# THUDM/GCC

Measured on NVIDIA H100. Metric: subgraphs/sec (MoCo pretrain step), higher is better.
Workload: dtype f32

## Files before the change

gcc_b200/csrc/posenc.cu:

```cuda
#include "common.cuh"

#include <stdlib.h>

namespace gccb {

#define GCCB_EIG_MAXSWEEP 14
#define GCCB_CF_B 48
#ifndef GCCB_CF_DEG0
#define GCCB_CF_DEG0 8
#endif
#ifndef GCCB_CF_DEG
#define GCCB_CF_DEG 16
#endif
#define GCCB_CF_LOGGAIN 19.1138f
#define GCCB_CF_MARGIN 0.05f
#define GCCB_CF_MARGIN_BELOW 0.25f
#ifndef GCCB_CF_SWEEPS0
#define GCCB_CF_SWEEPS0 0
#endif
#ifndef GCCB_CF_SWEEPS0_CLUSTER
#define GCCB_CF_SWEEPS0_CLUSTER 1
#endif
#define GCCB_DN_A 96
#define GCCB_DN_B 144
#define GCCB_DN_C 228
#define GCCB_CF_NSM 160
#define GCCB_CF_NSM_C 384
#define GCCB_CF_NSM_D1 1536
#define GCCB_CF_NSM_D 3584
#ifndef GCCB_CAP_MID2
#define GCCB_CAP_MID2 (GCCB_NUM_SMS * 2)
#endif
#ifndef GCCB_CAP_DN_A
#define GCCB_CAP_DN_A (GCCB_NUM_SMS * 4)
#endif
#ifndef GCCB_CAP_DN_B
#define GCCB_CAP_DN_B (GCCB_NUM_SMS * 2)
#endif
#ifndef GCCB_CAP_DN_C
#define GCCB_CAP_DN_C GCCB_NUM_SMS
#endif
#ifndef GCCB_BIG_NT
#define GCCB_BIG_NT 512
#endif
#define GCCB_CF_MAXIT 8
#define GCCB_GS_PANEL 4
#define GCCB_CF_TOL 4.0e-5f
#define GCCB_CF_STAG 2.0e-3f

#ifdef GCCB_EMU
#define GCCB_CLK() 0ll
#else
#define GCCB_CLK() clock64()
#endif
#define GCCB_TICK(k) do { if (threadIdx.x == 0) { long long t_ = GCCB_CLK(); ph[k] += t_ - t_last; t_last = t_; } } while (0)

#define GCCB_EIG_NCLASS 8
__device__ __forceinline__ int eig_class(int n, int dense_max) {
  if (n <= dense_max) return n <= GCCB_DN_A ? 0 : n <= GCCB_DN_B ? 1 : 2;
  return n <= GCCB_CF_NSM ? 3 : n <= GCCB_CF_NSM_C ? 4 : n <= GCCB_CF_NSM_D1 ? 5 : n <= GCCB_CF_NSM_D ? 6 : 7;
}

__global__ void __launch_bounds__(256)
posenc_classify_kernel(const int64_t* __restrict__ counters, const int32_t* __restrict__ node_off,
                       int B, int dense_max, int32_t* __restrict__ worklist, int32_t* __restrict__ counts) {
  __shared__ int scan_scratch[33];
  const int tid = threadIdx.x;
  int base[GCCB_EIG_NCLASS] = {0};
  for (int s0 = 0; s0 < 2 * B; s0 += 256) {
    int slot = s0 + tid;
    int cls = -1;
    if (slot < 2 * B) {
      int view = slot / B;
      if (node_off[view * (B + 1) + B] >= 0) cls = eig_class((int)counters[(size_t)slot * 4], dense_max);
    }
#pragma unroll
    for (int c = 0; c < GCCB_EIG_NCLASS; ++c) {
      int tot;
      int ex = block_scan_excl(cls == c ? 1 : 0, scan_scratch, &tot);
      if (cls == c) worklist[(size_t)c * 2 * B + base[c] + ex] = slot;
      base[c] += tot;
    }
  }
  if (tid < GCCB_EIG_NCLASS) counts[tid] = base[tid];
}

template <int NT>
__device__ __forceinline__ int jacobi_ritz48(float* A, float* V, float* cs , int* pq , int LD,
                                              float tol, int max_sweeps, long long* n_work = nullptr,
                                              long long* n_idle = nullptr) {
  constexpr int M = GCCB_CF_B, HALF = M / 2;
  const int tid = threadIdx.x;
  __shared__ float4 rec2[2][HALF];
  __shared__ int nrot2[2];
  (void)cs; (void)pq;
  for (int idx = tid; idx < M * M; idx += NT) {
    const int j = idx / M, i = idx - j * M;
    V[j * LD + i] = i == j ? 1.0f : 0.f;
  }
  __syncthreads();
  int sweep = 0;
  for (; sweep < max_sweeps; ++sweep) {
    if (max_sweeps > 1) {
      int any = 0;
      for (int idx = tid; idx < M * M; idx += NT) {
        const int q = idx / M, p = idx - q * M;
        if (p < q && fabsf(A[q * LD + p]) > tol * 0.5f * (fabsf(A[p * LD + p]) + fabsf(A[q * LD + q]))) any = 1;
// ... 990 lines not shown
    }
    if (tid == 0) {
      float w = 0.f, lo = theta[0], tk = theta[0];
      for (int c = 0; c < k; ++c) { w = fmaxf(w, resid[c]); tk = fminf(tk, theta[c]); }
      for (int i = 1; i < CB; ++i) lo = fminf(lo, theta[i]);
      if (tk < GCCB_CF_MARGIN_BELOW) lo = fminf(lo, tk - GCCB_CF_MARGIN);
      s_bc[0] = sqrtf(w);
      s_bc[1] = lo;
    }
    __syncthreads();
    const float w_all = s_bc[0];
    converged = (w_all < GCCB_CF_TOL) || (iter >= 2 && w_all < GCCB_CF_STAG && w_all > 0.5f * prev_worst);
    prev_worst = w_all;
    cut = fminf(fmaxf(s_bc[1], -0.9f), 0.95f);
    __syncthreads();
    GCCB_TICK(5);
  }
  if (C.rank == 0 && tid == 0) {
    if (!converged) atomicOr(flags, (int)GCCB_FLAG_EIG_NOCONV);
    dbg_iters[slot] = iter; dbg_res[slot] = prev_worst;
    for (int i = 0; i < 8; ++i) dbg_phase[(size_t)slot * 8 + i] = ph[i];
  }
  if (eigvals && C.rank == 0)
    for (int c = tid; c < pos_dim; c += NT) eigvals[(size_t)slot * pos_dim + c] = c < k ? theta[k - 1 - c] : 0.f;
  {
    float* best = part;
    for (int c = warp; c < k; c += NW) {
      float bb = -1.f, bval = 0.f; int brow = 0x7fffffff;
      for (int rl = lane; rl < nloc; rl += 32) {
        float x = X[(size_t)rl * ld + (k - 1 - c)], a = fabsf(x);
        if (a > bb) { bb = a; brow = r_lo + rl; bval = x; }
      }
#pragma unroll
      for (int o = 16; o > 0; o >>= 1) {
        float ob = __shfl_xor_sync(0xffffffffu, bb, o);
        int orow = __shfl_xor_sync(0xffffffffu, brow, o);
        float ov = __shfl_xor_sync(0xffffffffu, bval, o);
        if (ob > bb || (ob == bb && orow < brow)) { bb = ob; brow = orow; bval = ov; }
      }
      if (lane == 0) { best[c] = bb; best[48 + c] = __int_as_float(brow); best[96 + c] = bval; }
    }
    cl_sync<CS>();
    for (int c = tid; c < k; c += NT) {
      float bb = -1.f, bval = 0.f; int brow = 0x7fffffff;
      for (int q = 0; q < CS; ++q) {
        const float* rb = cl_map<CS>(best, q);
        float ob = rb[c]; int orow = __float_as_int(rb[48 + c]); float ov = rb[96 + c];
        if (ob > bb || (ob == bb && orow < brow)) { bb = ob; brow = orow; bval = ov; }
      }
      sgn[c] = bval < 0.f ? -1.0f : 1.0f;
    }
    __syncthreads();
  }
  float* out = pos + ((size_t)view * node_cap + noff) * pos_dim;
  for (int rl = warp; rl < nloc; rl += NW) {
    float u = 0.f;
    if (lane < k) u = sgn[lane] * X[(size_t)rl * ld + (k - 1 - lane)];
    if (normalize) {
      float ss = warp_sum(u * u);
      if (ss > 0.f) u = u / sqrtf(ss);
    }
    if (lane < pos_dim) out[(size_t)(r_lo + rl) * pos_dim + lane] = u;
  }
  cl_sync<CS>();
  }
}

#ifndef GCCB_DN_INVIT
#define GCCB_DN_INVIT 3
#endif
#ifndef GCCB_DN_MGS
#define GCCB_DN_MGS 1
#endif
#define GCCB_DN_PIVMIN 1.0e-30f
#define GCCB_DN_GUARD 1.0e-9f
#define GCCB_DN_TIGHT 2.0e-6f
#define GCCB_DN_DELTA 4.0e-6f
#define GCCB_DN_GAPTOL 1.0e-2f
#define GCCB_DN_RES_FLAG 1.0e-3f


__host__ __device__ constexpr int dn_ld(int n) { return ((n + 23) / 32) * 32 + 8; }

__device__ __forceinline__ int dn_sturm(const float* __restrict__ d, const float* __restrict__ e2, int n, float x) {
  float q = d[0] - x;
  if (fabsf(q) < GCCB_DN_PIVMIN) q = -GCCB_DN_PIVMIN;
  int c = q < 0.f ? 1 : 0;
  for (int i = 1; i < n; ++i) {
    q = (d[i] - x) - __fdividef(e2[i - 1], q);
    if (fabsf(q) < GCCB_DN_PIVMIN) q = -GCCB_DN_PIVMIN;
    c += q < 0.f ? 1 : 0;
  }
  return c;
}

template <int NMAX, int NT>
__device__ __forceinline__ void posenc_dense_item(const int slot, int B, int node_cap, int edge_cap,
                    const int32_t* __restrict__ node_off, const int32_t* __restrict__ b_indptr,
                    const int32_t* __restrict__ b_indices, const int32_t* __restrict__ sub_deg, int pos_dim, int normalize,
                    float* __restrict__ blocks, float* __restrict__ pos, float* __restrict__ eigvals,
                    int32_t* __restrict__ flags, int32_t* __restrict__ dbg_iters, float* __restrict__ dbg_res,
                    long long* __restrict__ dbg_phase) {
  constexpr int NW = NT / 32, NP = ((NMAX + 3) & ~3) + 4, NR = (NMAX + 31) / 32, CPW = 32 / NW;
  static_assert(NT >= 2 * NMAX && NW <= 32 && 32 % NW == 0, "two threads per matrix row");
  GCCB_DYN_SMEM(float, A);
  __align__(16) __shared__ float d[NP];
  __align__(16) __shared__ float e[NP];
  __align__(16) __shared__ float e2[NP];
  __align__(16) __shared__ float taus[NP];
  __align__(16) __shared__ float vbuf[NP];
  __align__(16) __shared__ float pbuf[NP];
  __align__(16) __shared__ float xbuf[NP];
  __align__(16) __shared__ float dinv[NP];
  __shared__ float ztail[32 * 32];
  __shared__ float lam[32], lamp[32], lo[32], hi[32], sgn[32];
  __shared__ int cnt[NT];
  __shared__ float part[NW * 32];
  long long ph[8] = {0, 0, 0, 0, 0, 0, 0, 0}, t_last = GCCB_CLK();
  const int view = slot / B, g = slot - view * B;
  const int noff = node_off[view * (B + 1) + g];
  const int n = node_off[view * (B + 1) + g + 1] - noff;
  const int tid = threadIdx.x, lane = tid & 31, warp = tid >> 5;
  const int k = min(n - 2, pos_dim);
  float* out = pos + ((size_t)view * node_cap + noff) * pos_dim;
  if (k <= 0) {
    for (int i = tid; i < n * pos_dim; i += NT) out[i] = 0.f;
    if (eigvals)
      for (int i = tid; i < pos_dim; i += NT) eigvals[(size_t)slot * pos_dim + i] = 0.f;
    if (tid == 0) { dbg_iters[slot] = 0; dbg_res[slot] = 0.f; }
    return;
  }
  const int ld = dn_ld(n);
  const int zb = n > 32 ? n - 32 : 0;
  auto zrow = [&](int i) -> float* { return i < zb ? A + (size_t)i * ld + (n - 32) : ztail + (i - zb) * 32; };
  const int32_t* v_indptr = b_indptr + (size_t)view * (node_cap + 1);
  const int32_t* v_indices = b_indices + (size_t)view * edge_cap;
  const int32_t* v_deg = sub_deg + (size_t)view * node_cap;
  float* U0 = blocks + ((size_t)view * node_cap + noff) * (GCCB_CF_B + 1);
  float* U1 = U0 + (size_t)2 * node_cap * (GCCB_CF_B + 1);
  for (int i = tid; i < NP; i += NT) { d[i] = 0.f; e[i] = 0.f; e2[i] = 0.f; taus[i] = 0.f; vbuf[i] = 0.f; pbuf[i] = 0.f; xbuf[i] = 0.f; }
  for (int i = tid; i < n; i += NT) {
    int dg = v_deg[noff + i];
    dinv[i] = 1.0f / sqrtf((float)(dg < 1 ? 1 : dg));
  }
  {
    float4* A4 = reinterpret_cast<float4*>(A);
    for (int i = tid; i < n * ld / 4; i += NT) A4[i] = make_float4(0.f, 0.f, 0.f, 0.f);
  }
  __syncthreads();
  for (int i = warp; i < n; i += NW) {
    const int beg = v_indptr[noff + i], end = v_indptr[noff + i + 1];
    const float di = dinv[i];
    for (int ed = beg + lane; ed < end; ed += 32) {
      int j = v_indices[ed] - noff;
      atomicAdd(&A[(size_t)j * ld + i], di * dinv[j]);
    }
  }
  __syncthreads();
  for (int i = tid; i < n; i += NT) xbuf[i] = i >= 1 ? A[(size_t)i * ld] : 0.f;
  __syncthreads();
  GCCB_TICK(0);
  {
    const int r = tid >> 1, h = tid & 1;
    float* row = A + (size_t)r * ld;
    for (int kk = 0; kk + 2 < n; ++kk) {
      const int c0 = (kk + 1) & ~3;
      const bool mine = r > kk && r < n;
      if (warp * 16 + 15 <= kk || warp * 16 >= n) {
        __syncthreads();
        __syncthreads();
        continue;
      }
      float y = 0.f;
      if (mine) {
        float y0 = 0.f, y1 = 0.f;
        int c = c0 + 4 * h;
        for (; c + 8 < n; c += 16) {
          const float4 a = *reinterpret_cast<const float4*>(row + c);
          const float4 x = *reinterpret_cast<const float4*>(xbuf + c);
          const float4 a2 = *reinterpret_cast<const float4*>(row + c + 8);
          const float4 x2 = *reinterpret_cast<const float4*>(xbuf + c + 8);
          y0 = fmaf(a.x, x.x, y0);
          y1 = fmaf(a.y, x.y, y1);
          y0 = fmaf(a.z, x.z, y0);
          y1 = fmaf(a.w, x.w, y1);
          y0 = fmaf(a2.x, x2.x, y0);
          y1 = fmaf(a2.y, x2.y, y1);
          y0 = fmaf(a2.z, x2.z, y0);
          y1 = fmaf(a2.w, x2.w, y1);
        }
        if (c < n) {
          const float4 a = *reinterpret_cast<const float4*>(row + c);
          const float4 x = *reinterpret_cast<const float4*>(xbuf + c);
          y0 = fmaf(a.x, x.x, y0);
          y1 = fmaf(a.y, x.y, y1);
          y0 = fmaf(a.z, x.z, y0);
          y1 = fmaf(a.w, x.w, y1);
        }
        y = y0 + y1;
      }
      y += __shfl_xor_sync(0xffffffffu, y, 1);
      float s = 0.f;
      for (int i = kk + 2 + lane; i < n; i += 32) { const float t = xbuf[i]; s = fmaf(t, t, s); }
      s = warp_sum(s);
      const float alpha = xbuf[kk + 1];
      float tau = 0.f, beta = alpha, scale = 0.f;
      if (s > 1.0e-30f) {
        beta = -copysignf(sqrtf(fmaf(alpha, alpha, s)), alpha);
        tau = (beta - alpha) / beta;
        scale = 1.0f / (alpha - beta);
      }
      if (mine && h == 0) {
        const float vr = r == kk + 1 ? 1.0f : xbuf[r] * scale;
        vbuf[r] = vr;
        pbuf[r] = tau * scale * (y - beta * row[kk + 1]);
        row[kk] = vr;
      }
      if (tid == 2 * (kk + 1)) {
        vbuf[kk] = 0.f; pbuf[kk] = 0.f;
        d[kk] = A[(size_t)kk * ld + kk]; e[kk] = beta; taus[kk] = tau;
      }
      __syncthreads();
      if (tau != 0.f) {
        float gs = 0.f;
        for (int i = kk + 1 + lane; i < n; i += 32) gs = fmaf(pbuf[i], vbuf[i], gs);
        const float gam = 0.5f * tau * warp_sum(gs);
        if (mine) {
          const float vr = vbuf[r], wr = fmaf(-gam, vr, pbuf[r]);
          const float nvr = -vr, nwr = -wr;
          auto upd = [&](float4& a, const float4& v4, const float4& p4) {
            a.x = fmaf(nwr, v4.x, fmaf(nvr, fmaf(-gam, v4.x, p4.x), a.x));
            a.y = fmaf(nwr, v4.y, fmaf(nvr, fmaf(-gam, v4.y, p4.y), a.y));
            a.z = fmaf(nwr, v4.z, fmaf(nvr, fmaf(-gam, v4.z, p4.z), a.z));
            a.w = fmaf(nwr, v4.w, fmaf(nvr, fmaf(-gam, v4.w, p4.w), a.w));
          };
          int c = c0 + 4 * h;
          for (; c + 8 < n; c += 16) {
            float4 a = *reinterpret_cast<float4*>(row + c);
            const float4 v4 = *reinterpret_cast<const float4*>(vbuf + c);
            const float4 p4 = *reinterpret_cast<const float4*>(pbuf + c);
            float4 a2 = *reinterpret_cast<float4*>(row + c + 8);
            const float4 v42 = *reinterpret_cast<const float4*>(vbuf + c + 8);
            const float4 p42 = *reinterpret_cast<const float4*>(pbuf + c + 8);
            upd(a, v4, p4);
            upd(a2, v42, p42);
            *reinterpret_cast<float4*>(row + c) = a;
            *reinterpret_cast<float4*>(row + c + 8) = a2;
          }
          if (c < n) {
            float4 a = *reinterpret_cast<float4*>(row + c);
            const float4 v4 = *reinterpret_cast<const float4*>(vbuf + c);
            const float4 p4 = *reinterpret_cast<const float4*>(pbuf + c);
            upd(a, v4, p4);
            *reinterpret_cast<float4*>(row + c) = a;
          }
        }
      }
      if (r > kk + 1 && r < n && h == 0) xbuf[r] = row[kk + 1];
      if (tid == 2 * (kk + 1)) xbuf[kk + 1] = 0.f;
      __syncthreads();
    }
    if (tid == 0) {
      d[n - 2] = A[(size_t)(n - 2) * ld + n - 2];
      d[n - 1] = A[(size_t)(n - 1) * ld + n - 1];
      e[n - 2] = A[(size_t)(n - 1) * ld + n - 2];
    }
    __syncthreads();
    for (int i = tid; i + 1 < n; i += NT) e2[i] = e[i] * e[i];
    __syncthreads();
  }
  GCCB_TICK(1);
  {
    float gl = 3.0e38f, gu = -3.0e38f;
    for (int i = lane; i < n; i += 32) {
      const float rad = (i > 0 ? fabsf(e[i - 1]) : 0.f) + (i + 1 < n ? fabsf(e[i]) : 0.f);
      gl = fminf(gl, d[i] - rad);
      gu = fmaxf(gu, d[i] + rad);
    }
    gl = -warp_max(-gl); gu = warp_max(gu);
    { const float pad = 1.0e-5f * fmaxf(fabsf(gl), fabsf(gu)) + 1.0e-6f; gl -= pad; gu += pad; }
    const float w0 = (gu - gl) / (float)(NT + 1);
    cnt[tid] = dn_sturm(d, e2, n, gl + (float)(tid + 1) * w0);
    __syncthreads();
    if (tid < k) {
      const int want = n - k + tid + 1;
      int a = 0, b = NT;
      while (a < b) { const int mid = (a + b) >> 1; if (cnt[mid] >= want) b = mid; else a = mid + 1; }
      hi[tid] = a < NT ? gl + (float)(a + 1) * w0 : gu;
      lo[tid] = a > 0 ? gl + (float)a * w0 : gl;
    }
    __syncthreads();
    constexpr int P = NT / 32;
    constexpr int ROUNDS = P >= 16 ? 4 : 5;
    const int j = tid / P, p = tid % P;
    const int want = n - k + j + 1;
    for (int rd = 0; rd < ROUNDS; ++rd) {
      float l = 0.f, wd = 0.f;
      int ok = 0;
      if (j < k) {
        l = lo[j];
        wd = (hi[j] - l) / (float)(P + 1);
        ok = dn_sturm(d, e2, n, l + (float)(p + 1) * wd) >= want;
      }
      const unsigned bal = __ballot_sync(0xffffffffu, ok);
      const unsigned grp = (bal >> (lane & ~(P - 1))) & ((1u << P) - 1u);
      __syncwarp();
      if (j < k && p == 0) {
        const int first = grp ? __ffs((int)grp) - 1 : P;
        if (first < P) hi[j] = l + (float)(first + 1) * wd;
        if (first > 0) lo[j] = l + (float)first * wd;
      }
      __syncwarp();
    }
    __syncthreads();
    if (tid < 32) lam[tid] = tid < k ? 0.5f * (lo[tid] + hi[tid]) : 0.f;
    __syncthreads();
    if (tid == 0) {
      int c = 0;
      while (c < k) {
        int ce = c;
        while (ce + 1 < k && lam[ce + 1] - lam[ce] < GCCB_DN_TIGHT) ++ce;
        if (ce > c) {
          const float below = c > 0 ? lam[c] - lam[c - 1] : 0.f;
          const float above = ce + 1 < k ? lam[ce + 1] - lam[ce] : 1.0f;
          const bool up = above >= below;
          const float dl = fminf(GCCB_DN_DELTA, (up ? above : below) * (1.0f / 3.0f));
          const float sh = up ? lam[ce] + dl : lam[c] - dl;
          for (int q = c; q <= ce; ++q) lamp[q] = sh;
        } else {
          lamp[c] = lam[c];
        }
        c = ce + 1;
      }
    }
    for (int i = tid; i < n * 32; i += NT) {
      const int r_ = i >> 5, c_ = i & 31;
      float v = 0.f;
      if (c_ < k) {
        u32x4 w = philox4x32_10((uint32_t)i, (uint32_t)n, 0x51ED270Bu, 7u, 0xC0FFEEu, 0x5EEDu);
        v = (float)(int32_t)w.x * (1.0f / 2147483648.0f);
      }
      zrow(r_)[c_] = v;
    }
    __syncthreads();
  }
  GCCB_TICK(2);
  for (int stage = 0; stage < 2; ++stage) {
  if (warp == 0 && lane < k) {
// ... 43 lines not shown
        }
        eb[0] = e[ib + 1];
#pragma unroll
        for (int q = 0; q < 4; ++q) {
          const int i = ib - q;
          if (i >= 0) {
            float ri = f0[q], u1 = f1[q], u2 = 0.f;
            if (ri == 0.f) { ri = __fdividef(1.0f, eb[q + 1]); u1 = db[q] - lj; u2 = eb[q]; }
            const float x = (bb[q] - u1 * x1 - u2 * x2) * ri;
            zrow(i)[j] = x;
            mx = fmaxf(mx, fabsf(x));
            x2 = x1; x1 = x;
          }
        }
#pragma unroll
        for (int q = 0; q < 4; ++q) { f0[q] = g0[q]; f1[q] = g1[q]; g0[q] = h0[q]; g1[q] = h1[q]; }
        ib -= 4;
      }
      if (!(mx > 0.f && mx < 3.0e38f)) {
        for (int i = 0; i < n; ++i) zrow(i)[j] = i == (j % n) ? 1.f : 0.f;
        mx = 1.f;
        atomicOr(flags, (int)GCCB_FLAG_EIG_NOCONV);
      }
      bscale = 1.0f / mx;
    }
    for (int i = 0; i < n; ++i) zrow(i)[j] *= bscale;
  }
  __syncthreads();
  GCCB_TICK(3);
  for (int pass = 0; pass < (stage == 0 ? 1 : GCCB_DN_MGS); ++pass)
    for (int j = k - 1; j >= 1; --j) {
      if (!(lam[j] - lam[j - 1] < GCCB_DN_GAPTOL)) continue;
      float acc = 0.f;
      for (int i0 = warp; i0 < n; i0 += 4 * NW) {
        float zj[4], zc[4];
#pragma unroll
        for (int q = 0; q < 4; ++q) {
          const int i = i0 + q * NW;
          const float* zr = zrow(i < n ? i : i0);
          zj[q] = i < n ? zr[j] : 0.f;
          zc[q] = zr[lane];
        }
#pragma unroll
        for (int q = 0; q < 4; ++q) acc = fmaf(zj[q], zc[q], acc);
      }
      part[warp * 32 + lane] = acc;
      __syncthreads();
      float dot = 0.f, nn = 0.f;
#pragma unroll
      for (int w = 0; w < NW; ++w) { dot += part[w * 32 + lane]; nn += part[w * 32 + j]; }
      const float coef = dot / fmaxf(nn, 1.0e-30f);
      if (lane < j)
        for (int i0 = warp; i0 < n; i0 += 4 * NW) {
          float zj[4], zc[4];
#pragma unroll
          for (int q = 0; q < 4; ++q) {
            const int i = i0 + q * NW;
            const float* zr = zrow(i < n ? i : i0);
            zj[q] = zr[j];
            zc[q] = zr[lane];
          }
#pragma unroll
          for (int q = 0; q < 4; ++q) {
            const int i = i0 + q * NW;
            if (i < n) zrow(i)[lane] = fmaf(-coef, zj[q], zc[q]);
          }
        }
      __syncthreads();
    }
  if (stage == 1) {
    float acc = 0.f;
    for (int i = warp; i < n; i += NW) { const float t = zrow(i)[lane]; acc = fmaf(t, t, acc); }
    part[warp * 32 + lane] = acc;
    __syncthreads();
    float nn = 0.f;
#pragma unroll
    for (int w = 0; w < NW; ++w) nn += part[w * 32 + lane];
    const float inv = 1.0f / sqrtf(fmaxf(nn, 1.0e-30f));
    for (int i = warp; i < n; i += NW) zrow(i)[lane] *= inv;
    __syncthreads();
  }
  GCCB_TICK(4);
  }
  {
    float xr[CPW][NR];
#pragma unroll
    for (int t = 0; t < NR; ++t) {
      const int rr = lane + 32 * t;
#pragma unroll
      for (int q = 0; q < CPW; ++q) xr[q][t] = rr < n ? zrow(rr)[warp * CPW + q] : 0.f;
    }
    for (int kk = n - 3; kk >= 0; --kk) {
      const float tau = taus[kk];
      if (tau == 0.f) continue;
      float vv[NR];
#pragma unroll
      for (int t = 0; t < NR; ++t) {
        const int rr = lane + 32 * t;
        vv[t] = (rr > kk && rr < n) ? A[(size_t)rr * ld + kk] : 0.f;
      }
#pragma unroll
      for (int q = 0; q < CPW; ++q) {
        float dt = 0.f;
#pragma unroll
        for (int t = 0; t < NR; ++t) dt = fmaf(vv[t], xr[q][t], dt);
        dt = tau * warp_sum(dt);
#pragma unroll
        for (int t = 0; t < NR; ++t) xr[q][t] = fmaf(-dt, vv[t], xr[q][t]);
      }
    }
    __syncthreads();
#pragma unroll
    for (int t = 0; t < NR; ++t) {
      const int rr = lane + 32 * t;
      if (rr < n) {
#pragma unroll
        for (int q = 0; q < CPW; ++q) zrow(rr)[warp * CPW + q] = xr[q][t];
      }
    }
    __syncthreads();
  }
  GCCB_TICK(5);
  {
    float acc = 0.f;
    const float lc = lam[lane];
    for (int i = warp; i < n; i += NW) {
      const int beg = v_indptr[noff + i], end = v_indptr[noff + i + 1];
      float yv = 0.f;
      for (int ed = beg; ed < end; ++ed) {
        const int jn = v_indices[ed] - noff;
        yv = fmaf(dinv[jn], zrow(jn)[lane], yv);
      }
      const float rs = fmaf(dinv[i], yv, -lc * zrow(i)[lane]);
      acc = fmaf(rs, rs, acc);
    }
    part[warp * 32 + lane] = acc;
    __syncthreads();
    if (warp == 0) {
      float tot = 0.f;
#pragma unroll
      for (int w = 0; w < NW; ++w) tot += part[w * 32 + lane];
      tot = lane < k ? tot : 0.f;
      tot = sqrtf(warp_max(tot));
      if (lane == 0) {
        dbg_iters[slot] = 0; dbg_res[slot] = tot;
        if (!(tot < GCCB_DN_RES_FLAG)) atomicOr(flags, (int)GCCB_FLAG_EIG_NOCONV);
        for (int i = 0; i < 8; ++i) dbg_phase[(size_t)slot * 8 + i] = ph[i];
      }
    }
  }
  if (eigvals)
    for (int c = tid; c < pos_dim; c += NT) eigvals[(size_t)slot * pos_dim + c] = c < k ? lam[c] : 0.f;
  write_features(n, k, pos_dim, normalize, sgn, out, [&](int c, int r_) { return zrow(r_)[c]; });
}

template <int NMAX, int NT>
__global__ void __launch_bounds__(NT, 65536 / 64 / NT)
posenc_dense_kernel(const int32_t* __restrict__ worklist , const int32_t* __restrict__ count,
                    int B, int node_cap, int edge_cap, const int32_t* __restrict__ node_off,
                    const int32_t* __restrict__ b_indptr, const int32_t* __restrict__ b_indices,
                    const int32_t* __restrict__ sub_deg, int pos_dim, int normalize, float* __restrict__ blocks,
                    float* __restrict__ pos, float* __restrict__ eigvals, int32_t* __restrict__ flags,
                    int32_t* __restrict__ dbg_iters, float* __restrict__ dbg_res, long long* __restrict__ dbg_phase) {
  for (int item = blockIdx.x; item < count[0]; item += gridDim.x) {
    posenc_dense_item<NMAX, NT>(worklist[item], B, node_cap, edge_cap, node_off, b_indptr, b_indices, sub_deg, pos_dim,
                                normalize, blocks, pos, eigvals, flags, dbg_iters, dbg_res, dbg_phase);
    __syncthreads();
  }
}

}

using namespace gccb;

static size_t posenc_ws_head(int B) {
  const size_t bytes = (size_t)2 * B * (8 * sizeof(long long) + sizeof(int32_t) + sizeof(float)) +
                       ((size_t)GCCB_EIG_NCLASS * 2 * B + GCCB_EIG_NCLASS) * sizeof(int32_t);
  return (bytes + 255) & ~(size_t)255;
}

extern "C" size_t gccb_posenc_workspace(int32_t batch, int32_t node_cap) {
  return posenc_ws_head(batch) + ((size_t)2 * node_cap + (size_t)2 * 2 * node_cap * (GCCB_CF_B + 1)) * sizeof(float);
}

static int posenc_dense_max() {
  const char* e = getenv("GCCB200_DENSE_MAX");
  const int v = e && e[0] ? atoi(e) : GCCB_DN_A;
  return v < GCCB_DN_A ? GCCB_DN_A : v > GCCB_DN_C ? GCCB_DN_C : v;
}

extern "C" int gccb_posenc(const gccb_batch_t* batch, int32_t pos_dim, int32_t normalize,
                           float* pos, float* eigvals, void* workspace, size_t workspace_bytes,
                           gccb_stream_t stream) {
  if (!batch || !pos || !workspace || batch->batch <= 0 || pos_dim < 2 || pos_dim > 32) {
    set_last_error("gccb_posenc: bad argument (pos_dim must be in [2, 32])");
    return GCCB_ERR_BADARG;
  }
  if ((uintptr_t)workspace % sizeof(long long)) {
    set_last_error("gccb_posenc: workspace must be 8-byte aligned");
    return GCCB_ERR_BADARG;
  }
  const int B = batch->batch;
  if (workspace_bytes < gccb_posenc_workspace(B, batch->node_cap)) {
    set_last_error("gccb_posenc: workspace too small");
    return GCCB_ERR_CAPACITY;
  }
  long long* dbg_phase = (long long*)workspace;
  int32_t* dbg_iters = (int32_t*)(dbg_phase + (size_t)2 * B * 8);
  float* dbg_res = (float*)(dbg_iters + (size_t)2 * B);
  int32_t* worklist = (int32_t*)(dbg_res + (size_t)2 * B);
  int32_t* counts = worklist + (size_t)GCCB_EIG_NCLASS * 2 * B;
  float* dinv = (float*)((char*)workspace + posenc_ws_head(B));
  float* blocks = dinv + (size_t)2 * batch->node_cap;
  const int dense_max = posenc_dense_max();
  GCCB_LAUNCH(posenc_classify_kernel, 1, 256, 0, stream, batch->counters, batch->node_off, B, dense_max, worklist,
              counts);
  auto kgiant = posenc_chfsi_kernel<0, 1024>;
#ifndef GCCB_EMU
  constexpr int CLUSTER = 8;
#else
  constexpr int CLUSTER = 1;
#endif
  auto khuge = posenc_chfsi_cluster_kernel<GCCB_BIG_NT, CLUSTER>;
  auto kbig = posenc_chfsi_kernel<1, GCCB_BIG_NT>;
  auto kmid = posenc_chfsi_kernel<1, 256>;
  auto kd_a = posenc_dense_kernel<GCCB_DN_A, 256>;
  auto kd_b = posenc_dense_kernel<GCCB_DN_B, 512>;
  auto kd_c = posenc_dense_kernel<GCCB_DN_C, 512>;
  const size_t s_b = (size_t)2 * GCCB_CF_NSM * (GCCB_CF_B + 1) * sizeof(float);
  const size_t s_c = (size_t)2 * GCCB_CF_NSM_C * (GCCB_CF_B + 1) * sizeof(float);
  const size_t s_d = (size_t)2 * ((GCCB_CF_NSM_D + CLUSTER - 1) / CLUSTER) * (GCCB_CF_B + 1) * sizeof(float);
  const size_t s_d1 = (size_t)2 * ((GCCB_CF_NSM_D1 + CLUSTER - 1) / CLUSTER) * (GCCB_CF_B + 1) * sizeof(float);
  const size_t sd_a = (size_t)GCCB_DN_A * dn_ld(GCCB_DN_A) * sizeof(float);
  const size_t sd_b = (size_t)GCCB_DN_B * dn_ld(GCCB_DN_B) * sizeof(float);
  const size_t sd_c = (size_t)GCCB_DN_C * dn_ld(GCCB_DN_C) * sizeof(float);
  gccb::ensure_dyn_smem(kmid, s_b);
  gccb::ensure_dyn_smem(kbig, s_c);
  gccb::ensure_dyn_smem(khuge, s_d);
  gccb::ensure_dyn_smem(kd_a, sd_a);
  gccb::ensure_dyn_smem(kd_b, sd_b);
  gccb::ensure_dyn_smem(kd_c, sd_c);
#ifndef GCCB_EMU
  StreamKit* kit = stream_kit((cudaStream_t)stream, 0, SidePriority::kLowest);
  cudaStream_t* side = kit->side;
  cudaEvent_t ev_fork = kit->ev[5];
  cudaEvent_t* ev_join = kit->ev;
  cudaStream_t main_s = (cudaStream_t)stream;
  cudaEventRecord(ev_fork, main_s);
  for (int i = 0; i < 4; ++i) cudaStreamWaitEvent(side[i], ev_fork, 0);
  gccb_stream_t s_giant = side[3], s_huge = side[0], s_big = side[1], s_mid = side[2];
#else
  gccb_stream_t s_giant = stream, s_huge = stream, s_big = stream, s_mid = stream;
#endif
#define GCCB_PE_ARGS(cls) worklist, counts, cls, B, batch->node_cap, batch->edge_cap, batch->node_off, batch->indptr, \
    batch->indices, batch->sub_deg, pos_dim, normalize, blocks, dinv, pos, eigvals, batch->flags, dbg_iters, dbg_res, dbg_phase
  auto capped = [&](int limit) { return 2 * B < limit ? 2 * B : limit; };
  GCCB_LAUNCH(kgiant, capped(8), 1024, 0, s_giant, GCCB_PE_ARGS(7));
  for (int pass = 0; pass < 2; ++pass) {
    const int cls = pass == 0 ? 5 : 6;
    const size_t smem = pass == 0 ? s_d1 : s_d;
    const int items = capped(pass == 0 ? 8 : 4);
    gccb_stream_t st = pass == 0 ? s_huge : s_giant;
#ifndef GCCB_EMU
    cudaLaunchConfig_t cfg = {};
    cfg.gridDim = dim3(CLUSTER * items); cfg.blockDim = dim3(GCCB_BIG_NT); cfg.dynamicSmemBytes = smem;
    cfg.stream = (cudaStream_t)st;
    cudaLaunchAttribute at[1];
    at[0].id = cudaLaunchAttributeClusterDimension;
    at[0].val.clusterDim.x = CLUSTER; at[0].val.clusterDim.y = 1; at[0].val.clusterDim.z = 1;
    cfg.attrs = at; cfg.numAttrs = 1;
    ++gccb::g_launch_count;
    cudaLaunchKernelEx(&cfg, khuge, (const int32_t*)worklist, (const int32_t*)counts, cls, B, batch->node_cap,
                       batch->edge_cap, (const int32_t*)batch->node_off, (const int32_t*)batch->indptr,
                       (const int32_t*)batch->indices, (const int32_t*)batch->sub_deg, pos_dim, normalize, dinv, pos,
                       eigvals, batch->flags, dbg_iters, dbg_res, dbg_phase);
#else
    GCCB_LAUNCH(khuge, items, GCCB_BIG_NT, smem, st, worklist, counts, cls, B, batch->node_cap, batch->edge_cap,
                batch->node_off, batch->indptr, batch->indices, batch->sub_deg, pos_dim, normalize, dinv, pos,
                eigvals, batch->flags, dbg_iters, dbg_res, dbg_phase);
#endif
  }
#define GCCB_DN_ARGS(c) worklist + (size_t)(c) * 2 * B, counts + (c), B, batch->node_cap, batch->edge_cap, \
    batch->node_off, batch->indptr, batch->indices, batch->sub_deg, pos_dim, normalize, blocks, pos, eigvals, \
    batch->flags, dbg_iters, dbg_res, dbg_phase
  if (dense_max > GCCB_DN_B) GCCB_LAUNCH(kd_c, capped(GCCB_CAP_DN_C), 512, sd_c, s_big, GCCB_DN_ARGS(2));
  if (dense_max > GCCB_DN_A) GCCB_LAUNCH(kd_b, capped(GCCB_CAP_DN_B), 512, sd_b, s_mid, GCCB_DN_ARGS(1));
  GCCB_LAUNCH(kd_a, capped(GCCB_CAP_DN_A), 256, sd_a, stream, GCCB_DN_ARGS(0));
  GCCB_LAUNCH(kbig, capped(GCCB_NUM_SMS), GCCB_BIG_NT, s_c, s_big, GCCB_PE_ARGS(4));
  if (dense_max < GCCB_CF_NSM) GCCB_LAUNCH(kmid, capped(GCCB_CAP_MID2), 256, s_b, s_mid, GCCB_PE_ARGS(3));
#ifndef GCCB_EMU
  for (int i = 0; i < 4; ++i) {
    cudaEventRecord(ev_join[i], side[i]);
    cudaStreamWaitEvent(main_s, ev_join[i], 0);
  }
#endif
  return check_launch("gccb_posenc");
}
```

profiles/dense_sanitize.py:

```python
#!/usr/bin/env python
import ctypes as C
import os
import sys

import numpy as np

ROOT = os.path.dirname(os.path.dirname(os.path.abspath(__file__)))
sys.path.insert(0, ROOT)
sys.path.insert(0, os.path.join(ROOT, "tests"))
from gcc_b200 import _capi
from gcc_b200.datasets import synthetic
from oracle import posenc as opos

os.environ["GCCB200_DENSE_MAX"] = "228"
rt = C.CDLL("/usr/local/cuda/lib64/libcudart.so")
rt.cudaMalloc.argtypes = [C.POINTER(C.c_void_p), C.c_size_t]
rt.cudaMemcpy.argtypes = [C.c_void_p, C.c_void_p, C.c_size_t, C.c_int]
rt.cudaMemset.argtypes = [C.c_void_p, C.c_int, C.c_size_t]
lib = _capi.bind(C.CDLL(os.path.join(ROOT, "gcc_b200", "libgccb200.so")))


def dev(a):
    p = C.c_void_p()
    assert rt.cudaMalloc(C.byref(p), max(a.nbytes, 8)) == 0
    assert rt.cudaMemcpy(p, a.ctypes.data_as(C.c_void_p), a.nbytes, 1) == 0
    return p


def host(p, like):
    out = np.empty_like(like)
    assert rt.cudaMemcpy(out.ctypes.data_as(C.c_void_p), p, out.nbytes, 2) == 0
    return out


def main():
    import emu_util
    small = len(sys.argv) > 1 and sys.argv[1] == "small"
    graphs = [synthetic.path_graph(5), synthetic.star_graph(33), synthetic.chung_lu(100, 250, seed=1),
              synthetic.erdos_renyi(34, 60, seed=2)]
    if not small:
        graphs += [synthetic.chung_lu(150, 400, seed=2), synthetic.star_graph(200), synthetic.erdos_renyi(228, 2000, seed=3),
                   synthetic.chung_lu(320, 900, exponent=0.7, seed=4)]
    subs = [dict(subv=np.arange(g.num_nodes, dtype=np.int32), indptr=g.indptr.astype(np.int32),
                 indices=g.indices.astype(np.int32), n=g.num_nodes, m=len(g.indices)) for g in graphs]
    half = len(subs) // 2
    views = [subs[:half], subs[half:]]
    emu_util.lib = lambda: None
    nb = emu_util.NpBatch.from_subgraphs(views)
    d = {k: dev(getattr(nb, k)) for k in ("node_off", "edge_off", "indptr", "indices", "sub_deg", "graph_id", "orig_id",
                                          "counters", "flags")}
    batch = _capi.Batch(nb.B, nb.node_cap, nb.edge_cap, 0, d["node_off"], d["edge_off"], d["indptr"], d["indices"],
                        d["sub_deg"], d["graph_id"], d["orig_id"], d["counters"], d["flags"])
    pos = np.zeros((2, nb.node_cap, 32), np.float32)
    eig = np.zeros((2 * nb.B, 32), np.float32)
    ws = np.zeros(lib.gccb_posenc_workspace(nb.B, nb.node_cap), np.uint8)
    dpos, deig, dws = dev(pos), dev(eig), dev(ws)
    rc = lib.gccb_posenc(C.byref(batch), 32, 0, dpos, deig, dws, ws.nbytes, None)
    assert rc == 0, lib.gccb_last_error()
    assert rt.cudaDeviceSynchronize() == 0
    pos, eig = host(dpos, pos), host(deig, eig)
    flags = host(d["flags"], nb.flags)
    worst = 0.0
    for v in (0, 1):
        for gi, s in enumerate(views[v]):
            a, z = nb.node_off[v, gi], nb.node_off[v, gi + 1]
            n = s["n"]
            k = min(n - 2, 32)
            lap = opos.normalized_adjacency(s["indptr"], s["indices"], n).toarray()
            w, _ = opos.eig_topk_exact(lap, k)
            theta, resid, ortho = opos.spectral_report(lap, pos[v, a:z, :k].astype(np.float64))
            bar = 2e-5 if n <= 228 else 2.5e-3
            assert np.abs(eig[v * nb.B + gi, :k] - w).max() < (2e-6 if n <= 228 else 1e-3) and resid.max() < bar and ortho < 1e-4, (
                n, np.abs(eig[v * nb.B + gi, :k] - w).max(), resid.max(), ortho)
            worst = max(worst, resid.max())
    print("dense_sanitize ok: %d ego-nets, flags %d, worst residual %.2e" % (len(subs), int(flags[0]), worst))


if __name__ == "__main__":
    main()
```

profiles/eig_dense_diag.py:

```python
#!/usr/bin/env python
import ctypes as C
import os
import sys

import numpy as np
import torch

sys.path.insert(0, os.path.dirname(os.path.dirname(os.path.abspath(__file__))))
import bench
from gcc_b200 import _lib
from gcc_b200.datasets.graph_dataset import LoadBalanceGraphDataset

cfg = bench.CONFIGS[sys.argv[1] if len(sys.argv) > 1 else "c2"]
dev = torch.device("cuda")
g = bench.make_graph_device(cfg, dev)
B = cfg["batch"]
ds = LoadBalanceGraphDataset(rw_hops=cfg["rw_hops"], restart_prob=0.8, dgl_graphs_file=g, batch_size=B, seed=0)
lib = _lib.get()
ev = [torch.cuda.Event(enable_timing=True) for _ in range(2)]


def posenc(buf, dense_max):
    if dense_max is None:
        os.environ.pop("GCCB200_DENSE_MAX", None)
    else:
        os.environ["GCCB200_DENSE_MAX"] = str(dense_max)
    ev[0].record()
    _lib.check(lib.gccb_posenc(C.byref(buf.c), 32, 1, _lib.dptr(buf.pos), _lib.dptr(buf.eigvals),
                               _lib.dptr(buf.ws_posenc), buf.ws_posenc.numel(), _lib.stream_ptr()))
    ev[1].record()
    torch.cuda.synchronize()
    return ev[0].elapsed_time(ev[1])


variants = [("dense<=228", 228), ("dense<=96", None)]
tot = {k: [] for k, _ in variants}
for st in range(int(sys.argv[2]) if len(sys.argv) > 2 else 8):
    buf = ds.sample_batch(posenc=False)
    torch.cuda.synchronize()
    for name, dm in variants:
        posenc(buf, dm)
        tot[name].append(min(posenc(buf, dm) for _ in range(2)))
    flags = int(buf.flags.item())
    buf.flags.zero_()
    n = buf.counters[:, 0].cpu().numpy()
    print("batch %d: largest n %s, flags %d, posenc ms %s" % (
        st, sorted(n.tolist())[-3:], flags, ", ".join("%s %.2f" % (k, tot[k][-1]) for k, _ in variants)))
print("mean posenc ms per batch: " + ", ".join("%s %.3f" % (k, np.mean(v)) for k, v in tot.items()))
posenc(buf, 228)
it, res = buf.eig_debug()
it, res = it.cpu().numpy(), res.cpu().numpy()
ph = buf.eig_phases().cpu().numpy()
n = buf.counters[:, 0].cpu().numpy()
names = ["setup", "tridiagonalisation", "multisection", "inverse iteration", "gram-schmidt", "back-transformation"]
for lo, hi in ((0, 96), (96, 144), (144, 228)):
    m = (n > lo) & (n <= hi) & (it == 0)
    if m.sum():
        t = ph[m][:, :6].sum(0).astype(float)
        print("dense n in (%d,%d]: %d ego-nets, cycles/ego-net %.0f k; split %s; kernel-side residual max %.1e" % (
            lo, hi, m.sum(), t.sum() / m.sum() / 1e3, ", ".join("%s %.0f%%" % (nm, 100 * x / t.sum()) for nm, x in zip(names, t)),
            res[m].max()))
```

Baseline: 235,200.

## Pack lower-triangular matrix in shared memory for mid and large dense eigensolvers

For the mid and large dense tiers, the symmetric matrix is now stored as a packed lower triangle with bank-staggered row offsets instead of a full padded square. The packed path uses one thread per row and 256 threads instead of two threads per row and 512. The upper-triangle part of each matrix-vector product is gathered column-wise through a row-offset table, and back-transformation processes half the columns per pass to save registers. The mid tier bound rises to 160. The aim is to cut shared memory per block so more blocks fit per SM, at the cost of strided gathers and fewer threads per row in the Householder tridiagonalisation.

```diff
diff --git a/gcc_b200/csrc/posenc.cu b/gcc_b200/csrc/posenc.cu
--- a/gcc_b200/csrc/posenc.cu
+++ b/gcc_b200/csrc/posenc.cu
@@ -22,7 +22,7 @@
 #define GCCB_CF_SWEEPS0_CLUSTER 1
 #endif
 #define GCCB_DN_A 96
-#define GCCB_DN_B 144
+#define GCCB_DN_B 160
 #define GCCB_DN_C 228
 #define GCCB_CF_NSM 160
 #define GCCB_CF_NSM_C 384
@@ -1179,6 +1179,20 @@
 
 __host__ __device__ constexpr int dn_ld(int n) { return ((n + 23) / 32) * 32 + 8; }
 
+__host__ __device__ constexpr int dn_pk_off(int r) {
+  int cur = 0;
+  unsigned used = 0;
+  for (int i = 0;; ++i) {
+    if ((i & 7) == 0) used = 0;
+    while ((used >> (cur & 7)) & 1u) ++cur;
+    if (i == r) return 4 * cur;
+    used |= 1u << (cur & 7);
+    cur += (i + 4) >> 2;
+  }
+}
+#define GCCB_DN_ZLD 33
+__host__ __device__ constexpr int dn_pk_floats(int nmax) { return dn_pk_off(nmax) + nmax * GCCB_DN_ZLD; }
+
 __device__ __forceinline__ int dn_sturm(const float* __restrict__ d, const float* __restrict__ e2, int n, float x) {
   float q = d[0] - x;
   if (fabsf(q) < GCCB_DN_PIVMIN) q = -GCCB_DN_PIVMIN;
@@ -1197,9 +1211,10 @@
                     const int32_t* __restrict__ b_indices, const int32_t* __restrict__ sub_deg, int pos_dim, int normalize,
                     float* __restrict__ blocks, float* __restrict__ pos, float* __restrict__ eigvals,
                     int32_t* __restrict__ flags, int32_t* __restrict__ dbg_iters, float* __restrict__ dbg_res,
-                    long long* __restrict__ dbg_phase) {
+                    long long* __restrict__ dbg_phase, const int* __restrict__ roff ) {
   constexpr int NW = NT / 32, NP = ((NMAX + 3) & ~3) + 4, NR = (NMAX + 31) / 32, CPW = 32 / NW;
-  static_assert(NT >= 2 * NMAX && NW <= 32 && 32 % NW == 0, "two threads per matrix row");
+  constexpr bool PACKED = NT < 2 * NMAX;
+  static_assert(NT >= (PACKED ? 1 : 2) * NMAX && NW <= 32 && 32 % NW == 0, "threads per matrix row");
   GCCB_DYN_SMEM(float, A);
   __align__(16) __shared__ float d[NP];
   __align__(16) __shared__ float e[NP];
@@ -1209,7 +1224,7 @@
   __align__(16) __shared__ float pbuf[NP];
   __align__(16) __shared__ float xbuf[NP];
   __align__(16) __shared__ float dinv[NP];
-  __shared__ float ztail[32 * 32];
+  __shared__ float ztail[PACKED ? 1 : 32 * 32];
   __shared__ float lam[32], lamp[32], lo[32], hi[32], sgn[32];
   __shared__ int cnt[NT];
   __shared__ float part[NW * 32];
@@ -1229,7 +1244,14 @@
   }
   const int ld = dn_ld(n);
   const int zb = n > 32 ? n - 32 : 0;
-  auto zrow = [&](int i) -> float* { return i < zb ? A + (size_t)i * ld + (n - 32) : ztail + (i - zb) * 32; };
+  auto amat = [&](int r_, int c_) -> float& {
+    if constexpr (PACKED) return A[roff[r_] + c_];
+    else return A[(size_t)r_ * ld + c_];
+  };
+  auto zrow = [&](int i) -> float* {
+    if constexpr (PACKED) return A + dn_pk_off(NMAX) + i * GCCB_DN_ZLD;
+    else return i < zb ? A + (size_t)i * ld + (n - 32) : ztail + (i - zb) * 32;
+  };
   const int32_t* v_indptr = b_indptr + (size_t)view * (node_cap + 1);
   const int32_t* v_indices = b_indices + (size_t)view * edge_cap;
   const int32_t* v_deg = sub_deg + (size_t)view * node_cap;
@@ -1242,7 +1264,8 @@
   }
   {
     float4* A4 = reinterpret_cast<float4*>(A);
-    for (int i = tid; i < n * ld / 4; i += NT) A4[i] = make_float4(0.f, 0.f, 0.f, 0.f);
+    const int n4 = PACKED ? roff[n] / 4 : n * ld / 4;
+    for (int i = tid; i < n4; i += NT) A4[i] = make_float4(0.f, 0.f, 0.f, 0.f);
   }
   __syncthreads();
   for (int i = warp; i < n; i += NW) {
@@ -1250,14 +1273,14 @@
     const float di = dinv[i];
     for (int ed = beg + lane; ed < end; ed += 32) {
       int j = v_indices[ed] - noff;
-      atomicAdd(&A[(size_t)j * ld + i], di * dinv[j]);
+      if (!PACKED || j >= i) atomicAdd(&amat(j, i), di * dinv[j]);
     }
   }
   __syncthreads();
-  for (int i = tid; i < n; i += NT) xbuf[i] = i >= 1 ? A[(size_t)i * ld] : 0.f;
+  for (int i = tid; i < n; i += NT) xbuf[i] = i >= 1 ? amat(i, 0) : 0.f;
   __syncthreads();
   GCCB_TICK(0);
-  {
+  if constexpr (!PACKED) {
     const int r = tid >> 1, h = tid & 1;
     float* row = A + (size_t)r * ld;
     for (int kk = 0; kk + 2 < n; ++kk) {
@@ -1357,10 +1380,155 @@
       if (tid == 2 * (kk + 1)) xbuf[kk + 1] = 0.f;
       __syncthreads();
     }
+  } else {
+    const int r = tid;
+    float* row = A + roff[r < NMAX ? r : NMAX];
+    const int rl = r & ~3;
+    __shared__ float2 xo[NMAX];
+    for (int i = tid; i < n; i += NT) xo[i] = make_float2(xbuf[i], __int_as_float(roff[i]));
+    __syncthreads();
+    for (int kk = 0; kk + 2 < n; ++kk) {
+      const int c0 = (kk + 1) & ~3;
+      const bool mine = r > kk && r < n;
+      if (warp * 32 + 31 <= kk || warp * 32 >= n) {
+        __syncthreads();
+        __syncthreads();
+        continue;
+      }
+      float y = 0.f;
+      if (mine) {
+        float y0 = 0.f, y1 = 0.f, y2 = 0.f, y3 = 0.f;
+        int c = c0;
+        for (; c + 4 <= rl; c += 8) {
+          const float4 a = *reinterpret_cast<const float4*>(row + c);
+          const float4 x = *reinterpret_cast<const float4*>(xbuf + c);
+          const float4 a2 = *reinterpret_cast<const float4*>(row + c + 4);
+          const float4 x2 = *reinterpret_cast<const float4*>(xbuf + c + 4);
+          y0 = fmaf(a.x, x.x, y0);
+          y1 = fmaf(a.y, x.y, y1);
+          y0 = fmaf(a.z, x.z, y0);
+          y1 = fmaf(a.w, x.w, y1);
+          y0 = fmaf(a2.x, x2.x, y0);
+          y1 = fmaf(a2.y, x2.y, y1);
+          y0 = fmaf(a2.z, x2.z, y0);
+          y1 = fmaf(a2.w, x2.w, y1);
+        }
+        if (c <= rl) {
+          const float4 a = *reinterpret_cast<const float4*>(row + c);
+          const float4 x = *reinterpret_cast<const float4*>(xbuf + c);
+          y0 = fmaf(a.x, x.x, y0);
+          y1 = fmaf(a.y, x.y, y1);
+          y0 = fmaf(a.z, x.z, y0);
+          y1 = fmaf(a.w, x.w, y1);
+        }
+        c = n - 1;
+        for (; c - 7 > r; c -= 8) {
+          float2 q[8];
+          float a[8];
+#pragma unroll
+          for (int i = 0; i < 8; ++i) q[i] = xo[c - i];
+#pragma unroll
+          for (int i = 0; i < 8; ++i) a[i] = A[__float_as_int(q[i].y) + r];
+#pragma unroll
+          for (int i = 0; i < 8; i += 2) { y2 = fmaf(a[i], q[i].x, y2); y3 = fmaf(a[i + 1], q[i + 1].x, y3); }
+        }
+        if (c - 3 > r) {
+          float2 q[4];
+          float a[4];
+#pragma unroll
+          for (int i = 0; i < 4; ++i) q[i] = xo[c - i];
+#pragma unroll
+          for (int i = 0; i < 4; ++i) a[i] = A[__float_as_int(q[i].y) + r];
+#pragma unroll
+          for (int i = 0; i < 4; i += 2) { y2 = fmaf(a[i], q[i].x, y2); y3 = fmaf(a[i + 1], q[i + 1].x, y3); }
+          c -= 4;
+        }
+        for (; c > r; --c) { const float2 q = xo[c]; y2 = fmaf(A[__float_as_int(q.y) + r], q.x, y2); }
+        y = (y0 + y1) + (y2 + y3);
+      }
+      float s = 0.f;
+      for (int i = kk + 2 + lane; i < n; i += 32) { const float t = xbuf[i]; s = fmaf(t, t, s); }
+      s = warp_sum(s);
+      const float alpha = xbuf[kk + 1];
+      float tau = 0.f, beta = alpha, scale = 0.f;
+      if (s > 1.0e-30f) {
+        beta = -copysignf(sqrtf(fmaf(alpha, alpha, s)), alpha);
+        tau = (beta - alpha) / beta;
+        scale = 1.0f / (alpha - beta);
+      }
+      if (mine) {
+        const float vr = r == kk + 1 ? 1.0f : xbuf[r] * scale;
+        vbuf[r] = vr;
+        pbuf[r] = tau * scale * (y - beta * row[kk + 1]);
+        row[kk] = vr;
+      }
+      if (tid == kk + 1) {
+        vbuf[kk] = 0.f; pbuf[kk] = 0.f;
+        d[kk] = amat(kk, kk); e[kk] = beta; taus[kk] = tau;
+      }
+      __syncthreads();
+      if (tau != 0.f) {
+        float gs = 0.f;
+        for (int i = kk + 1 + lane; i < n; i += 32) gs = fmaf(pbuf[i], vbuf[i], gs);
+        const float gam = 0.5f * tau * warp_sum(gs);
+        if (mine) {
+          const float vr = vbuf[r], wr = fmaf(-gam, vr, pbuf[r]);
+          const float nvr = -vr, nwr = -wr;
+          auto upd = [&](float4& a, const float4& v4, const float4& p4) {
+            a.x = fmaf(nwr, v4.x, fmaf(nvr, fmaf(-gam, v4.x, p4.x), a.x));
+            a.y = fmaf(nwr, v4.y, fmaf(nvr, fmaf(-gam, v4.y, p4.y), a.y));
+            a.z = fmaf(nwr, v4.z, fmaf(nvr, fmaf(-gam, v4.z, p4.z), a.z));
+            a.w = fmaf(nwr, v4.w, fmaf(nvr, fmaf(-gam, v4.w, p4.w), a.w));
+          };
+          int c = c0;
+          for (; c + 4 < rl; c += 8) {
+            float4 a = *reinterpret_cast<float4*>(row + c);
+            const float4 v4 = *reinterpret_cast<const float4*>(vbuf + c);
+            const float4 p4 = *reinterpret_cast<const float4*>(pbuf + c);
+            float4 a2 = *reinterpret_cast<float4*>(row + c + 4);
+            const float4 v42 = *reinterpret_cast<const float4*>(vbuf + c + 4);
+            const float4 p42 = *reinterpret_cast<const float4*>(pbuf + c + 4);
+            upd(a, v4, p4);
+            upd(a2, v42, p42);
+            *reinterpret_cast<float4*>(row + c) = a;
+            *reinterpret_cast<float4*>(row + c + 4) = a2;
+          }
+          if (c < rl) {
+            float4 a = *reinterpret_cast<float4*>(row + c);
+            const float4 v4 = *reinterpret_cast<const float4*>(vbuf + c);
+            const float4 p4 = *reinterpret_cast<const float4*>(pbuf + c);
+            upd(a, v4, p4);
+            *reinterpret_cast<float4*>(row + c) = a;
+          }
+          {
+            float4 a = *reinterpret_cast<float4*>(row + rl);
+            float4 v4 = *reinterpret_cast<const float4*>(vbuf + rl);
+            float4 p4 = *reinterpret_cast<const float4*>(pbuf + rl);
+            const int m = r - rl;
+            if (m < 1) { v4.y = 0.f; p4.y = 0.f; }
+            if (m < 2) { v4.z = 0.f; p4.z = 0.f; }
+            if (m < 3) { v4.w = 0.f; p4.w = 0.f; }
+            upd(a, v4, p4);
+            *reinterpret_cast<float4*>(row + rl) = a;
+          }
+        }
+      }
+      if (r > kk + 1 && r < n) { const float xn = row[kk + 1]; xbuf[r] = xn; xo[r].x = xn; }
+      if (tid == kk + 1) { xbuf[kk + 1] = 0.f; xo[kk + 1].x = 0.f; }
+      __syncthreads();
+    }
+  }
+  {
     if (tid == 0) {
-      d[n - 2] = A[(size_t)(n - 2) * ld + n - 2];
-      d[n - 1] = A[(size_t)(n - 1) * ld + n - 1];
-      e[n - 2] = A[(size_t)(n - 1) * ld + n - 2];
+      if constexpr (PACKED) {
+        d[n - 2] = amat(n - 2, n - 2);
+        d[n - 1] = amat(n - 1, n - 1);
+        e[n - 2] = amat(n - 1, n - 2);
+      } else {
+        d[n - 2] = A[(size_t)(n - 2) * ld + n - 2];
+        d[n - 1] = A[(size_t)(n - 1) * ld + n - 1];
+        e[n - 2] = A[(size_t)(n - 1) * ld + n - 2];
+      }
     }
     __syncthreads();
     for (int i = tid; i + 1 < n; i += NT) e2[i] = e[i] * e[i];
@@ -1570,13 +1738,15 @@
   }
   GCCB_TICK(4);
   }
-  {
-    float xr[CPW][NR];
+  constexpr int QP = PACKED ? CPW / 2 : CPW;
+#pragma unroll 1
+  for (int q0 = 0; q0 < CPW; q0 += QP) {
+    float xr[QP][NR];
 #pragma unroll
     for (int t = 0; t < NR; ++t) {
       const int rr = lane + 32 * t;
 #pragma unroll
-      for (int q = 0; q < CPW; ++q) xr[q][t] = rr < n ? zrow(rr)[warp * CPW + q] : 0.f;
+      for (int q = 0; q < QP; ++q) xr[q][t] = rr < n ? zrow(rr)[warp * CPW + q0 + q] : 0.f;
     }
     for (int kk = n - 3; kk >= 0; --kk) {
       const float tau = taus[kk];
@@ -1585,10 +1755,10 @@
 #pragma unroll
       for (int t = 0; t < NR; ++t) {
         const int rr = lane + 32 * t;
-        vv[t] = (rr > kk && rr < n) ? A[(size_t)rr * ld + kk] : 0.f;
-      }
-#pragma unroll
-      for (int q = 0; q < CPW; ++q) {
+        vv[t] = (rr > kk && rr < n) ? amat(rr, kk) : 0.f;
+      }
+#pragma unroll
+      for (int q = 0; q < QP; ++q) {
         float dt = 0.f;
 #pragma unroll
         for (int t = 0; t < NR; ++t) dt = fmaf(vv[t], xr[q][t], dt);
@@ -1603,7 +1773,7 @@
       const int rr = lane + 32 * t;
       if (rr < n) {
 #pragma unroll
-        for (int q = 0; q < CPW; ++q) zrow(rr)[warp * CPW + q] = xr[q][t];
+        for (int q = 0; q < QP; ++q) zrow(rr)[warp * CPW + q0 + q] = xr[q][t];
       }
     }
     __syncthreads();
@@ -1650,10 +1820,21 @@
                     const int32_t* __restrict__ sub_deg, int pos_dim, int normalize, float* __restrict__ blocks,
                     float* __restrict__ pos, float* __restrict__ eigvals, int32_t* __restrict__ flags,
                     int32_t* __restrict__ dbg_iters, float* __restrict__ dbg_res, long long* __restrict__ dbg_phase) {
-  for (int item = blockIdx.x; item < count[0]; item += gridDim.x) {
-    posenc_dense_item<NMAX, NT>(worklist[item], B, node_cap, edge_cap, node_off, b_indptr, b_indices, sub_deg, pos_dim,
-                                normalize, blocks, pos, eigvals, flags, dbg_iters, dbg_res, dbg_phase);
-    __syncthreads();
+  if constexpr (NT < 2 * NMAX) {
+    __shared__ int roff[NMAX + 1];
+    for (int r = threadIdx.x; r <= NMAX; r += NT) roff[r] = dn_pk_off(r);
+    __syncthreads();
+    for (int item = blockIdx.x; item < count[0]; item += gridDim.x) {
+      posenc_dense_item<NMAX, NT>(worklist[item], B, node_cap, edge_cap, node_off, b_indptr, b_indices, sub_deg,
+                                  pos_dim, normalize, blocks, pos, eigvals, flags, dbg_iters, dbg_res, dbg_phase, roff);
+      __syncthreads();
+    }
+  } else {
+    for (int item = blockIdx.x; item < count[0]; item += gridDim.x) {
+      posenc_dense_item<NMAX, NT>(worklist[item], B, node_cap, edge_cap, node_off, b_indptr, b_indices, sub_deg,
+                                  pos_dim, normalize, blocks, pos, eigvals, flags, dbg_iters, dbg_res, dbg_phase, nullptr);
+      __syncthreads();
+    }
   }
 }
 
@@ -1713,15 +1894,15 @@
   auto kbig = posenc_chfsi_kernel<1, GCCB_BIG_NT>;
   auto kmid = posenc_chfsi_kernel<1, 256>;
   auto kd_a = posenc_dense_kernel<GCCB_DN_A, 256>;
-  auto kd_b = posenc_dense_kernel<GCCB_DN_B, 512>;
-  auto kd_c = posenc_dense_kernel<GCCB_DN_C, 512>;
+  auto kd_b = posenc_dense_kernel<GCCB_DN_B, 256>;
+  auto kd_c = posenc_dense_kernel<GCCB_DN_C, 256>;
   const size_t s_b = (size_t)2 * GCCB_CF_NSM * (GCCB_CF_B + 1) * sizeof(float);
   const size_t s_c = (size_t)2 * GCCB_CF_NSM_C * (GCCB_CF_B + 1) * sizeof(float);
   const size_t s_d = (size_t)2 * ((GCCB_CF_NSM_D + CLUSTER - 1) / CLUSTER) * (GCCB_CF_B + 1) * sizeof(float);
   const size_t s_d1 = (size_t)2 * ((GCCB_CF_NSM_D1 + CLUSTER - 1) / CLUSTER) * (GCCB_CF_B + 1) * sizeof(float);
   const size_t sd_a = (size_t)GCCB_DN_A * dn_ld(GCCB_DN_A) * sizeof(float);
-  const size_t sd_b = (size_t)GCCB_DN_B * dn_ld(GCCB_DN_B) * sizeof(float);
-  const size_t sd_c = (size_t)GCCB_DN_C * dn_ld(GCCB_DN_C) * sizeof(float);
+  const size_t sd_b = (size_t)dn_pk_floats(GCCB_DN_B) * sizeof(float);
+  const size_t sd_c = (size_t)dn_pk_floats(GCCB_DN_C) * sizeof(float);
   gccb::ensure_dyn_smem(kmid, s_b);
   gccb::ensure_dyn_smem(kbig, s_c);
   gccb::ensure_dyn_smem(khuge, s_d);
@@ -1771,8 +1952,8 @@
 #define GCCB_DN_ARGS(c) worklist + (size_t)(c) * 2 * B, counts + (c), B, batch->node_cap, batch->edge_cap, \
     batch->node_off, batch->indptr, batch->indices, batch->sub_deg, pos_dim, normalize, blocks, pos, eigvals, \
     batch->flags, dbg_iters, dbg_res, dbg_phase
-  if (dense_max > GCCB_DN_B) GCCB_LAUNCH(kd_c, capped(GCCB_CAP_DN_C), 512, sd_c, s_big, GCCB_DN_ARGS(2));
-  if (dense_max > GCCB_DN_A) GCCB_LAUNCH(kd_b, capped(GCCB_CAP_DN_B), 512, sd_b, s_mid, GCCB_DN_ARGS(1));
+  if (dense_max > GCCB_DN_B) GCCB_LAUNCH(kd_c, capped(GCCB_CAP_DN_C), 256, sd_c, s_big, GCCB_DN_ARGS(2));
+  if (dense_max > GCCB_DN_A) GCCB_LAUNCH(kd_b, capped(GCCB_CAP_DN_B), 256, sd_b, s_mid, GCCB_DN_ARGS(1));
   GCCB_LAUNCH(kd_a, capped(GCCB_CAP_DN_A), 256, sd_a, stream, GCCB_DN_ARGS(0));
   GCCB_LAUNCH(kbig, capped(GCCB_NUM_SMS), GCCB_BIG_NT, s_c, s_big, GCCB_PE_ARGS(4));
   if (dense_max < GCCB_CF_NSM) GCCB_LAUNCH(kmid, capped(GCCB_CAP_MID2), 256, s_b, s_mid, GCCB_PE_ARGS(3));
diff --git a/profiles/dense_sanitize.py b/profiles/dense_sanitize.py
--- a/profiles/dense_sanitize.py
+++ b/profiles/dense_sanitize.py
@@ -40,6 +40,7 @@
               synthetic.erdos_renyi(34, 60, seed=2)]
     if not small:
         graphs += [synthetic.chung_lu(150, 400, seed=2), synthetic.star_graph(200), synthetic.erdos_renyi(228, 2000, seed=3),
+                   synthetic.star_graph(96), synthetic.star_graph(160),
                    synthetic.chung_lu(320, 900, exponent=0.7, seed=4)]
     subs = [dict(subv=np.arange(g.num_nodes, dtype=np.int32), indptr=g.indptr.astype(np.int32),
                  indices=g.indices.astype(np.int32), n=g.num_nodes, m=len(g.indices)) for g in graphs]
diff --git a/profiles/eig_dense_diag.py b/profiles/eig_dense_diag.py
--- a/profiles/eig_dense_diag.py
+++ b/profiles/eig_dense_diag.py
@@ -53,7 +53,7 @@
 ph = buf.eig_phases().cpu().numpy()
 n = buf.counters[:, 0].cpu().numpy()
 names = ["setup", "tridiagonalisation", "multisection", "inverse iteration", "gram-schmidt", "back-transformation"]
-for lo, hi in ((0, 96), (96, 144), (144, 228)):
+for lo, hi in ((0, 96), (96, 160), (160, 228)):
     m = (n > lo) & (n <= hi) & (it == 0)
     if m.sum():
         t = ph[m][:, :6].sum(0).astype(float)
```

Result: no change. 235,300 (median of 6 runs) (+0.1%).
